# zafarrafii/REPET-Python

Measured on AMD Instinct MI355X. Metric: audio-seconds/sec (x real-time) for repet.sim, 44.1 kHz stereo, higher is better.
Workload: dtype f32 (similarity GEMM: f16x3 split of the fp32 unit rows, fp32 accumulate; median: exact selection on bit-sliced rank codes)

## Files before the change

### repet-python_amd/csrc/rank.hip

```cpp
#include "common.h"

namespace repet {

namespace {

__device__ __forceinline__ void cex(unsigned& a, unsigned& b) {
    const unsigned lo = a < b ? a : b, hi = a < b ? b : a;
    a = lo; b = hi;
}
__device__ __forceinline__ int phys(int i) { return i + ((i >> 5) << 2); }

template <int QHI, int QLO, int HB>
__device__ __forceinline__ void stages_high(unsigned (&r)[8][4]) {
#pragma unroll
    for (int q = QHI; q >= QLO; --q) {
        const int bit = 1 << (q - HB);
#pragma unroll
        for (int u = 0; u < 8; ++u)
            if (!(u & bit)) {
#pragma unroll
                for (int w = 0; w < 4; ++w) cex(r[u][w], r[u | bit][w]);
            }
    }
}
// ... 13 lines not shown
            const int src = (i0 ^ ((1 << (P - 1)) - 1)) & ~3;
            const uint4 v = *reinterpret_cast<const uint4*>(s + phys(src));
            r[u][0] = v.w; r[u][1] = v.z; r[u][2] = v.y; r[u][3] = v.x;
        } else {
            const uint4 v = *reinterpret_cast<const uint4*>(s + phys(i0));
            r[u][0] = v.x; r[u][1] = v.y; r[u][2] = v.z; r[u][3] = v.w;
        }
    }
    if (FLIP) __syncthreads();
    stages_high<QHI, QLO, HB>(r);
#pragma unroll
    for (int u = 0; u < 8; ++u)
        *reinterpret_cast<uint4*>(s + phys(base | (u << HB))) = make_uint4(r[u][0], r[u][1], r[u][2], r[u][3]);
}

template <int LOG2N, int P, int QHI>
struct HighTrips {
    static __device__ __forceinline__ void run(unsigned* s, int tid) {
        constexpr int QLO = QHI - 2 > 5 ? QHI - 2 : 5;
        trip_high<LOG2N, P, QHI, QLO, QHI == P - 1>(s, tid);
        if constexpr (QLO > 5) HighTrips<LOG2N, P, QLO - 1>::run(s, tid);
    }
};

__device__ __forceinline__ void stages_low(unsigned (&k)[32]) {
#pragma unroll
    for (int q = 4; q >= 0; --q) {
#pragma unroll
        for (int i = 0; i < 32; ++i)
            if (!(i & (1 << q))) cex(k[i], k[i | (1 << q)]);
    }
}

__device__ __forceinline__ void load_run(const unsigned* s, int tid, unsigned (&k)[32]) {
#pragma unroll
    for (int v = 0; v < 8; ++v) {
        const uint4 x = *reinterpret_cast<const uint4*>(s + phys(tid * 32 + v * 4));
        k[4 * v] = x.x; k[4 * v + 1] = x.y; k[4 * v + 2] = x.z; k[4 * v + 3] = x.w;
    }
}
__device__ __forceinline__ void store_run(unsigned* s, int tid, const unsigned (&k)[32]) {
#pragma unroll
    for (int v = 0; v < 8; ++v)
        *reinterpret_cast<uint4*>(s + phys(tid * 32 + v * 4)) = make_uint4(k[4 * v], k[4 * v + 1], k[4 * v + 2], k[4 * v + 3]);
}

template <int LOG2N, int P>
struct Phases {
    static __device__ __forceinline__ void run(unsigned* s, int tid, unsigned (&k)[32]) {
        HighTrips<LOG2N, P, P - 1>::run(s, tid);
        __syncthreads();
        load_run(s, tid, k);
        stages_low(k);
        store_run(s, tid, k);
        if constexpr (P < LOG2N) Phases<LOG2N, P + 1>::run(s, tid, k);
    }
};

}

constexpr int kColumnTileFrames = 32;
__global__ __launch_bounds__(256) void columns_from_rows_kernel(RankArgs a) {
    constexpr int TF = kColumnTileFrames;
    constexpr int kRounds = TF / 16;
    constexpr int kOutLanes = TF / 4;
    constexpr int kOutRounds = 64 * kOutLanes / 256;
    __shared__ float tile[TF][65];
    const int c = blockIdx.z, f0 = blockIdx.y * 64;
    const int64_t t0 = (int64_t)blockIdx.x * TF;
    const int tx = threadIdx.x & 15, ty = threadIdx.x >> 4;
    const float* in = a.V + c * a.chan_stride;
    float4 r[kRounds];
#pragma unroll
    for (int k = 0; k < kRounds; ++k) {
        const int64_t t = t0 + ty + 16 * k;
        r[k] = *reinterpret_cast<const float4*>(in + (t < a.T ? t : a.T - 1) * a.FS + f0 + 4 * tx);
    }
#pragma unroll
    for (int k = 0; k < kRounds; ++k) {
        const bool live = t0 + ty + 16 * k < a.T;
        float* row = tile[ty + 16 * k] + 4 * tx;
        row[0] = live ? r[k].x : 0.f; row[1] = live ? r[k].y : 0.f; row[2] = live ? r[k].z : 0.f; row[3] = live ? r[k].w : 0.f;
    }
    __syncthreads();
    float* out = a.Vs + ((int64_t)c * a.n_cols + f0) * a.vs_pitch;
    const int ox = threadIdx.x % kOutLanes, oy = threadIdx.x / kOutLanes;
    const int col0 = (oy & 3) + 32 * ((oy >> 2) & 1) + 4 * (threadIdx.x >> 6);
    if (t0 + 4 * ox < a.vs_pitch) {
#pragma unroll
        for (int k = 0; k < kOutRounds; ++k) {
            const int f = col0 + 16 * k;
            *reinterpret_cast<float4*>(out + (int64_t)f * a.vs_pitch + t0 + 4 * ox) =
                make_float4(tile[4 * ox][f], tile[4 * ox + 1][f], tile[4 * ox + 2][f], tile[4 * ox + 3][f]);
        }
    }
}

__global__ __launch_bounds__(256) void rows_from_code_columns_kernel(RankArgs a) {
    __shared__ unsigned tile[2][64][65];
    const int c = blockIdx.z, f0 = blockIdx.y * 128;
    const int64_t t0 = (int64_t)blockIdx.x * 128;
    const int tx = threadIdx.x & 63, ty = threadIdx.x >> 6;
    const unsigned* in = reinterpret_cast<const unsigned*>(a.codes + ((int64_t)c * a.n_cols + f0) * a.vs_pitch + t0);
    const bool in_range = t0 + 2 * tx < a.vs_pitch;
    unsigned r[32];
    const int txc = in_range ? tx : 0;
#pragma unroll
    for (int k = 0; k < 32; ++k) r[k] = in[(int64_t)(ty + 4 * k) * (a.vs_pitch / 2) + txc];
// ... 21 lines not shown
    for (int k = 0; k < 16; ++k)
        if (!(k & J)) {
            const unsigned t = ((x[k] >> J) ^ x[k + J]) & m;
            x[k + J] ^= t;
            x[k] ^= t << J;
        }
}
constexpr int kPlaneFrames = 32;
__global__ __launch_bounds__(1024) void code_planes_from_columns_kernel(RankArgs a) {
    constexpr int kPlaneColPitch = kPlaneFrames + 2, kPieces = kPlaneFrames / 8;
    extern __shared__ unsigned short plane_lds[];
    const int64_t t0 = (int64_t)blockIdx.x * kPlaneFrames;
    const int l0 = blockIdx.y * 32;
    const int bpc = a.n_cols >> 6, n_bits = a.n_channels * bpc;
    uint4 v[kPieces];
#pragma unroll
    for (int k = 0; k < kPieces; ++k) {
        const int i = threadIdx.x + 1024 * k, q = i / kPieces, piece = i % kPieces;
        const int b = q >> 5, l = l0 + (q & 31);
        const int64_t t = t0 + piece * 8;
        const bool in = b < n_bits && t < a.vs_pitch;
        const int c = in ? b / bpc : 0, f = in ? (b - c * bpc) * 64 + l : 0;
        v[k] = *reinterpret_cast<const uint4*>(a.codes + ((int64_t)c * a.n_cols + f) * a.vs_pitch + (in ? t : 0));
        if (!in) v[k] = make_uint4(0u, 0u, 0u, 0u);
    }
#pragma unroll
    for (int k = 0; k < kPieces; ++k) {
        const int i = threadIdx.x + 1024 * k, q = i / kPieces, piece = i % kPieces;
        unsigned* dst = reinterpret_cast<unsigned*>(plane_lds + q * kPlaneColPitch + piece * 8);
        dst[0] = v[k].x; dst[1] = v[k].y; dst[2] = v[k].z; dst[3] = v[k].w;
    }
    __syncthreads();
    const int l = threadIdx.x & 31;
#pragma unroll
    for (int k = 0; k < kPlaneFrames / 32; ++k) {
        const int tl = (threadIdx.x >> 5) + 32 * k;
        const int64_t t = t0 + tl;
        if (t >= a.T) continue;
        unsigned x[16];
#pragma unroll
        for (int b = 0; b < 16; ++b) {
            const unsigned lo = b < n_bits ? plane_lds[(b * 32 + l) * kPlaneColPitch + tl] - kRankCodeBase : 0u;
            const unsigned hi = b + 16 < n_bits ? plane_lds[((b + 16) * 32 + l) * kPlaneColPitch + tl] - kRankCodeBase : 0u;
            x[b] = (lo & 0xffffu) | (hi << 16);
        }
        plane_transpose_stage<8>(x); plane_transpose_stage<4>(x); plane_transpose_stage<2>(x); plane_transpose_stage<1>(x);
        unsigned* out = a.P + t * (int64_t)a.n_planes * 64 + l0 + l;
#pragma unroll
        for (int p = 0; p < 15; ++p)
            if (p < a.n_planes) out[p * 64] = x[p];
    }
}

#ifndef REPET_RANK_LEAF_BITS
#define REPET_RANK_LEAF_BITS 4
#endif
constexpr int rank_leaf_bits(int log2n) { return log2n >= 15 ? 5 : REPET_RANK_LEAF_BITS; }

template <int LOG2N>
__global__ __launch_bounds__((1 << LOG2N) / 32) void rank_columns_kernel(RankArgs a) {
    constexpr int N = 1 << LOG2N, THREADS = N / 32;
    extern __shared__ uint4 rank_lds[];
    unsigned* s = reinterpret_cast<unsigned*>(rank_lds);
    const int64_t col = blockIdx.x;
    const int tid = threadIdx.x;
    float* column = a.Vs + col * a.vs_pitch;
    const __amdgpu_buffer_rsrc_t v_rsrc = __builtin_amdgcn_make_buffer_rsrc(column, 0, (int)(a.T * 4), 0x00020000);
    unsigned k[32];
#pragma unroll
    for (int j = 0; j < 8; ++j) {
        const int t = 4 * tid + 4 * THREADS * j;
        const uint4 v = __builtin_bit_cast(uint4, __builtin_amdgcn_raw_buffer_load_b128(v_rsrc, t * 4, 0, 0));
        k[4 * j] = t < a.T ? v.x : 0x7f800000u;
        k[4 * j + 1] = t + 1 < a.T ? v.y : 0x7f800000u;
        k[4 * j + 2] = t + 2 < a.T ? v.z : 0x7f800000u;
        k[4 * j + 3] = t + 3 < a.T ? v.w : 0x7f800000u;
    }
#pragma unroll
    for (int p = 1; p <= 5; ++p) {
#pragma unroll
        for (int i2 = 0; i2 < 32; ++i2)
            if (!(i2 & (1 << (p - 1)))) cex(k[i2], k[i2 ^ ((1 << p) - 1)]);
#pragma unroll
        for (int q = p - 2; q >= 0; --q) {
#pragma unroll
            for (int i2 = 0; i2 < 32; ++i2)
                if (!(i2 & (1 << q))) cex(k[i2], k[i2 | (1 << q)]);
        }
    }
    store_run(s, tid, k);
    Phases<LOG2N, 6>::run(s, tid, k);
    unsigned orig[32], pos[32];
#pragma unroll
    for (int j = 0; j < 8; ++j) {
        const int t = 4 * tid + 4 * THREADS * j;
        const uint4 v = __builtin_bit_cast(uint4, __builtin_amdgcn_raw_buffer_load_b128(v_rsrc, t * 4, 0, 0));
        orig[4 * j] = v.x; orig[4 * j + 1] = v.y; orig[4 * j + 2] = v.z; orig[4 * j + 3] = v.w;
    }
    constexpr int R = rank_leaf_bits(LOG2N), kTreeLevels = LOG2N - R, kNodes = N >> R;
    unsigned* tree = s + (N + N / 8);
    __syncthreads();
#pragma unroll
    for (int n = tid; n < kNodes; n += THREADS)
        if (n > 0) {
            const int l = 31 - __clz(n), j = n - (1 << l);
            tree[n] = s[phys((((2 * j + 1) << (LOG2N - 1 - l))) - 1)];
        }
    __syncthreads();
    {
#pragma unroll
        for (int e = 0; e < 32; ++e) pos[e] = 1;
#pragma unroll 1
        for (int l = 0; l < kTreeLevels; ++l) {
#pragma unroll
            for (int e = 0; e < 32; ++e) {
                const unsigned probe = tree[pos[e]];
                pos[e] = 2 * pos[e] + (probe < orig[e] ? 1 : 0);
            }
        }
#pragma unroll
        for (int e = 0; e < 32; ++e) {
            const int g = pos[e] - kNodes;
            pos[e] = (g << R) + ((g >> (5 - R)) << 2) + (1 << (R - 1)) - 1;
        }
#pragma unroll
        for (int m = R - 1; m >= 0; --m) {
            const int step = 1 << m, d = m > 0 ? -((step >> 1) + 0) : 0;
#pragma unroll
            for (int e = 0; e < 32; ++e) {
                const unsigned probe = s[pos[e]];
                pos[e] += (probe < orig[e] ? step : 0) + d;
            }
        }
    }
#pragma unroll
    for (int e = 0; e < 32; ++e) pos[e] -= 4 * (pos[e] / 36);
    const __amdgpu_buffer_rsrc_t c_rsrc = __builtin_amdgcn_make_buffer_rsrc(a.codes + col * a.vs_pitch, 0, (int)(round_up(a.T, 4) * 2), 0x00020000);
#pragma unroll
    for (int j = 0; j < 8; ++j) {
        const int t = 4 * tid + 4 * THREADS * j;
        const unsigned lo = (kRankCodeBase + pos[4 * j]) | ((kRankCodeBase + pos[4 * j + 1]) << 16);
        const unsigned hi = (kRankCodeBase + pos[4 * j + 2]) | ((kRankCodeBase + pos[4 * j + 3]) << 16);
        __builtin_amdgcn_raw_buffer_store_b64(__builtin_bit_cast(__attribute__((__vector_size__(2 * sizeof(unsigned)))) unsigned, make_uint2(lo, hi)),
                                              c_rsrc, t * 2, 0, 0);
    }
    __syncthreads();
#pragma unroll
    for (int j = 0; j < 8; ++j) {
        const int t = 4 * tid + 4 * THREADS * j;
        if (t < a.vs_pitch) *reinterpret_cast<uint4*>(column + t) = *reinterpret_cast<const uint4*>(s + phys(t));
    }
}

__global__ void fill_rank_pad_rows_kernel(unsigned short* R, int64_t r_chan_stride, int64_t pad_row, int FS) {
    const int c = blockIdx.y;
    const int k = blockIdx.x * blockDim.x + threadIdx.x;
    if (k >= 2 * FS) return;
    R[c * r_chan_stride + pad_row * FS + k] = (k < FS) ? (unsigned short)0 : (unsigned short)0x7C00;
}

hipError_t launch_fill_rank_pad_rows(unsigned short* R, int64_t r_chan_stride, int32_t n_channels, int64_t pad_row,
                                     int32_t FS, hipStream_t s) {
    hipLaunchKernelGGL(fill_rank_pad_rows_kernel, dim3((unsigned)ceil_div(2 * FS, 256), (unsigned)n_channels), dim3(256), 0, s,
                       R, r_chan_stride, pad_row, FS);
    return hipGetLastError();
}

bool rank_columns_supported(int64_t T) { return T > kRankMinFrames && T <= kRankMaxFrames; }

template <int LOG2N>
static hipError_t launch_rank_n(const RankArgs& a, hipStream_t s, RankStepHook hook, void* user) {
    constexpr int N = 1 << LOG2N;
    constexpr int lds = (N + N / 8) * 4 + (N >> rank_leaf_bits(LOG2N)) * 4;
    hipError_t e = ensure_dynamic_lds(reinterpret_cast<const void*>(&rank_columns_kernel<LOG2N>), lds);
    if (e != hipSuccess) return e;
    const int64_t cols = (int64_t)a.n_channels * a.n_cols;
    hipLaunchKernelGGL(columns_from_rows_kernel, dim3((unsigned)ceil_div(a.vs_pitch, kColumnTileFrames), (unsigned)(a.n_cols / 64), (unsigned)a.n_channels),
                       dim3(256), 0, s, a);
    if (hook) hook(user, 0);
    hipLaunchKernelGGL(rank_columns_kernel<LOG2N>, dim3((unsigned)cols), dim3(N / 32), lds, s, a);
    if (hook) hook(user, 1);
    if (a.P) {
        constexpr int plane_lds_bytes = 1024 * (kPlaneFrames + 2) * 2;
        e = ensure_dynamic_lds(reinterpret_cast<const void*>(&code_planes_from_columns_kernel), plane_lds_bytes);
        if (e != hipSuccess) return e;
        hipLaunchKernelGGL(code_planes_from_columns_kernel, dim3((unsigned)ceil_div(a.T, kPlaneFrames), 2), dim3(1024), plane_lds_bytes, s, a);
        if (hook) hook(user, 2);
        return hipGetLastError();
    }
    hipLaunchKernelGGL(rows_from_code_columns_kernel, dim3((unsigned)ceil_div(a.vs_pitch, 128), (unsigned)(a.n_cols / 128), (unsigned)a.n_channels),
                       dim3(256), 0, s, a);
    if (hook) hook(user, 3);
    return hipGetLastError();
}

hipError_t launch_rank_columns(const RankArgs& a0, hipStream_t s, RankStepHook hook, void* user) {
    if (!rank_columns_supported(a0.T) || a0.n_cols <= 0 || (a0.n_cols & 127) || (a0.vs_pitch & 31) || (a0.FS & 1)) return hipErrorInvalidValue;
    if (a0.P && (a0.R || a0.n_planes != code_planes_for(a0.T) || a0.n_planes > 15 || a0.n_channels * (a0.n_cols >> 6) > 32)) return hipErrorInvalidValue;
    if (!a0.P && !a0.R) return hipErrorInvalidValue;
    RankArgs a = a0;
    if (a.T <= 2048) return launch_rank_n<11>(a, s, hook, user);
    if (a.T <= 4096) return launch_rank_n<12>(a, s, hook, user);
    if (a.T <= 8192) return launch_rank_n<13>(a, s, hook, user);
    if (a.T <= 16384) return launch_rank_n<14>(a, s, hook, user);
    return launch_rank_n<15>(a, s, hook, user);
}

}
```

### repet-python_amd/csrc/common.h

```cpp
#pragma once
#include <hip/hip_runtime.h>
#include <stdint.h>
#include "../../include/repet_hip.h"
#include <vector>

namespace repet {

constexpr int kWave = 64;
constexpr int kFreqAlign = 32;
constexpr int kTile = 128;
constexpr float kMaskEps = 2.220446049250313e-16f;

__host__ __device__ inline int64_t round_up(int64_t x, int64_t m) { return (x + m - 1) / m * m; }
__host__ __device__ inline int64_t ceil_div(int64_t x, int64_t m) { return (x + m - 1) / m; }

hipError_t ensure_dynamic_lds(const void* kernel, int bytes);


struct StftArgs {
    const float* audio; int64_t n_samples; int32_t n_channels;
    int64_t sample_offset;
    const float* window; const float2* twiddle;
    int32_t W, H; int64_t T; int32_t FS; int32_t centred;
    float2* X; float* V; int64_t chan_stride;
// ... 163 lines not shown
hipError_t launch_unit_rows_f64(const struct ExactSource& src, const PeakRefine* refine, hipStream_t s);
size_t local_maxima_scratch_bytes(int64_t n_rows, int32_t n_cols, int32_t d);

struct ExactSource {
    const float* hi; const float* lo; int64_t n_samples; int32_t n_channels; int64_t clip_stride;
    int64_t frame_sample0; int32_t W, H, F, FS;
    const double* window64; const double2* twiddle64;
    double* u64; int64_t u64_clip_stride; unsigned int* u64_gen; int64_t gen_clip_stride;
};
size_t local_maxima_exact_scratch_bytes(int32_t n_cols, int* grid_out = nullptr);
hipError_t launch_local_maxima_exact(const float* M, int64_t row0, int32_t n_cols, int64_t pitch, int32_t mode, float min_value,
                                     int32_t d, int32_t number, int32_t* idx, int32_t idx_pitch, int32_t* count, hipStream_t s,
                                     int64_t shift, const PeakRefine* refine, const PeakBatch* batch, const ExactSource& src,
                                     void* scratch);

__device__ __forceinline__ float soft_mask(float v, float model, int f, int cutoff) {
#ifdef REPET_IEEE_SQRT
    const float m = (fminf(v, model) + kMaskEps) / (v + kMaskEps);
#else
    const float q = fminf((model + kMaskEps) * __builtin_amdgcn_rcpf(v + kMaskEps), 1.0f);
    const float m = (model >= v) ? 1.0f : q;
#endif
    const float mm = (model != model) ? model : m;
    return (f >= 1 && f <= cutoff) ? 1.0f : mm;
}

struct MaskArgs {
    const float* V; int64_t chan_stride; int32_t n_channels; int64_t T; int32_t F, FS;
    float2* X; float* mask; int32_t cutoff;
    float* model; int64_t model_batch_stride, model_chan_stride;
    int64_t pad_row;
    int32_t n_batch; int64_t batch_stride;
    int64_t idx_batch_stride, cnt_batch_stride;
    int64_t frame0;
    int64_t frame_end;
    const unsigned short* R; int64_t r_chan_stride; const float* Vs; int64_t vs_pitch; int32_t n_rank_cols;
    const unsigned* P; int32_t n_planes;
    unsigned* median_codes;
    const int64_t* slot_start; int64_t slot_bias;
};
constexpr int kPadRows = 8;
constexpr int kMinIdxPitch = 128;
hipError_t launch_fill_pad_rows(float* V, int64_t chan_stride, int32_t n_channels, int64_t pad_row, int32_t FS,
                                hipStream_t s, float* Z = nullptr, int64_t z_stride = 0, int64_t z_count = 0, int32_t n_z = 0,
                                unsigned int* stats = nullptr, float* Z2 = nullptr);
hipError_t launch_mask_sim(const MaskArgs& m, const int32_t* idx, int32_t idx_pitch, const int32_t* count,
                           int64_t first_frame, int32_t max_count, hipStream_t s, int parts = 3, bool lookups_by_caller = false);
int median_network_instructions(int max_n, int* net_size);
int code_planes_for(int64_t T);
bool mask_sim_bits_supported(int64_t T, int32_t n_channels, int32_t n_cols, int32_t max_count);
int mask_sim_bits_instructions(int32_t max_count, int32_t n_planes);
hipError_t launch_mask_sim_bits(const MaskArgs& m, const int32_t* idx, int32_t idx_pitch, const int32_t* count, int32_t max_count,
                                unsigned n_launch, hipStream_t s);
hipError_t launch_mask_from_codes(const MaskArgs& m, const int32_t* count, hipStream_t s);
hipError_t launch_mask_adaptive(const MaskArgs& m, const int32_t* periods, int32_t order, hipStream_t s);
hipError_t launch_mask_period(const MaskArgs& m, const int32_t* period_dev, int32_t period_host,
                              int32_t min_period, hipStream_t s);

constexpr int kRankCodeBase = 0x0400;
constexpr int kRankMinFrames = 1024;
constexpr int kRankMaxFrames = 30720;
struct RankArgs {
    const float* V; int64_t chan_stride; int32_t n_channels; int64_t T; int32_t FS;
    int32_t n_cols;
    unsigned short* R; int64_t r_chan_stride;
    float* Vs; int64_t vs_pitch;
    unsigned short* codes;
    unsigned* P; int32_t n_planes;
};
bool rank_columns_supported(int64_t T);
std::vector<int> host_cpus_near_device(int dev);
typedef void (*RankStepHook)(void* user, int step);
hipError_t launch_rank_columns(const RankArgs& a, hipStream_t s, RankStepHook hook = nullptr, void* user = nullptr);
hipError_t launch_fill_rank_pad_rows(unsigned short* R, int64_t r_chan_stride, int32_t n_channels, int64_t pad_row,
                                     int32_t FS, hipStream_t s);

struct StagingRing {
    static constexpr int kSlots = 6;
    static constexpr size_t kSlotElems = (size_t)1 << 20;
    float* base = nullptr;
    float* base_lo = nullptr;
    float* lo_full = nullptr; size_t lo_full_elems = 0; hipEvent_t hi_done = nullptr, lo_done = nullptr; bool lo_in_flight = false;
    hipEvent_t event[kSlots] = {};
    bool busy[kSlots] = {};
    hipError_t ensure();
    hipError_t ensure_lo();
    hipError_t ensure_lo_full(size_t elems);
    void release();
    ~StagingRing();
};
hipError_t staged_upload(StagingRing& ring, const void* src, int dtype, float* dst, size_t count, hipStream_t s,
                         float* dst_lo = nullptr, bool* any_lo = nullptr, hipStream_t s_lo = nullptr, bool* not_finite = nullptr);
hipError_t staged_download(StagingRing& ring, const float* src, double* dst, size_t count, hipStream_t s);
hipError_t staged_upload_bytes(StagingRing& ring, const void* src, void* dst, size_t n_bytes, hipStream_t s);
const char* wav_parse(const void* file, int64_t n_bytes, ::repet_wav_info* info);
int wav_itemsize(const ::repet_wav_info& w);
hipError_t launch_decode_pcm(const void* raw, int format, int width, float* dst, int64_t n, hipStream_t s);
int64_t wav_float_header(unsigned char* out, int sampling_frequency, int n_channels, int64_t n_samples, int item_bytes);
void* host_alloc(size_t bytes);
void host_free(void* ptr);

hipError_t launch_convert_in(const void* src, int dtype, float* dst, int64_t count, hipStream_t s, float* dst_lo = nullptr);
hipError_t launch_convert_out(const float* src, double* dst, int64_t count, hipStream_t s);
hipError_t launch_foreground(const float* audio, const float* background, double* dst, int64_t count, hipStream_t s);
hipError_t launch_foreground_f32(const float* audio, const float* background, float* dst, int64_t count, hipStream_t s);
hipError_t launch_channel_mean(const float* audio, const float* background, int which, int n_channels, float* dst,
                               int64_t n_samples, hipStream_t s);
// ... 5 lines not shown
```

### repet-python_amd/csrc/engine_sim.hip

```cpp
#include "engine.h"

using namespace repet;
using namespace repet_eng;

namespace repet_eng {

float peak_refine_delta(int FS, bool f16_gram) {
    return (f16_gram ? 2.0f : 4.0f) * sqrtf((float)FS) * 5.9604645e-8f;
}

double peak_exact_delta2() {
    static const double v = [] { const char* off = getenv("REPET_PEAK_EXACT"); return (off && off[0] == '0') ? 0.0 : 2.5e-7; }();
    return v;
}

int ensure_stamps(repet_ctx* c, DevBuf& buf, size_t count) {
    if (buf.cap >= count * sizeof(unsigned int)) return REPET_OK;
    HIP_TRY(hipStreamSynchronize(c->stream));
    HIP_TRY(buf.ensure(count * sizeof(unsigned int)));
    HIP_TRY(hipMemsetAsync(buf.p, 0, buf.cap, c->stream));
    return REPET_OK;
}

int make_refine(repet_ctx* c, const float* unit_rows, int FS, double threshold, PeakRefine* rf, int64_t rows, int clips,
// ... 120 lines not shown
    const int64_t TS = round_up(T, 64);
    HIP_TRY(c->S.ensure((size_t)T * TS * sizeof(float)));
    const bool with_seg = local_maxima_segments_apply((int)T, p->sim_distance_frames, TS, 0, 1);
    const int seg_pitch = segment_pitch((int)TS);
    if (with_seg) HIP_TRY(c->seg.ensure((size_t)T * 3 * seg_pitch * sizeof(float)));
    float* seg = with_seg ? c->seg.as<float>() : nullptr;
    bool seg_written = false;
    RP_TRY(run_gram_full(c, c->Vn.as<float>(), T, g.FS, c->S.as<float>(), TS, true, split_in_stft(1), seg, seg_pitch, &seg_written));
    {
        const bool f16 = gram_f16_enabled();
        const int edge = (f16 && gram_big_enabled() && T >= 8 * gram_big_tile()) ? gram_big_tile() : kTile;
        const double n_tiles = 0.5 * (double)ceil_div(T, edge) * (double)(ceil_div(T, edge) + 1);
        mark(c, f16 ? "similarity_gemm_f16x3" : "similarity_gemm", 4.0 * g.F * T + 4.0 * T * T,
             (f16 ? 3.0 : 1.0) * 2.0 * g.FS * n_tiles * edge * edge);
    }
    if (seg && !seg_written) {
        HIP_TRY(launch_segment_maxima(c->S.as<float>(), T, (int)T, TS, seg, seg_pitch, c->stream));
        mark(c, "segment_maxima", 4.0 * T * T + 12.0 * T * seg_pitch, 0);
    }
    const int K = p->sim_number, KP = std::max(K, kMinIdxPitch);
    HIP_TRY(c->idx.ensure((size_t)T * KP * sizeof(int32_t)));
    HIP_TRY(c->cnt.ensure((size_t)T * sizeof(int32_t)));
    PeakRefine rf{};
    RP_TRY(make_refine(c, c->Vn.as<float>(), g.FS, p->sim_threshold, &rf, T, 1, (int)T, p->sim_distance_frames, T));
    {
        MaskArgs m = mask_args(c, g, p->cutoff_bins);
        static const bool overlap = [] { const char* e = getenv("REPET_RANK_OVERLAP"); return !(e && e[0] == '0'); }();
        const bool beside = use_rank && overlap;
        if (beside) {
            HIP_TRY(hipEventRecord(c->fork_event, c->stream));
            HIP_TRY(hipStreamWaitEvent(c->side_stream, c->fork_event, 0));
            RP_TRY(run_rank_columns(c, g, &m, c->side_stream, false, max_peaks));
            HIP_TRY(hipEventRecord(c->join_event, c->side_stream));
        }
        const size_t scratch = local_maxima_scratch_bytes(T, (int)T, p->sim_distance_frames);
        if (scratch > 0) HIP_TRY(c->peak_scratch.ensure(scratch));
        hipError_t e = launch_local_maxima(c->S.as<float>(), T, 0, (int)T, TS, 0, (float)p->sim_threshold,
                                           p->sim_distance_frames, K, c->idx.as<int32_t>(), KP, c->cnt.as<int32_t>(), c->stream, 0, &rf,
                                           nullptr, scratch > 0 ? c->peak_scratch.p : nullptr, nullptr, seg, seg_pitch);
        if (e == hipErrorInvalidValue) return fail(REPET_ERR_LIMIT, "sim: clip has too many frames for the peak-picking kernel's LDS row");
        HIP_TRY(e);
        if (use_rank && !beside) mark(c, "local_maxima_pass1", 12.0 * T * seg_pitch + 4.0 * K * T, 0);
        RP_TRY(run_exact_rows(c, tb, g, c->S.as<float>(), 0, (int)T, TS, 0, (float)p->sim_threshold, p->sim_distance_frames, K,
                              c->idx.as<int32_t>(), KP, c->cnt.as<int32_t>(), 0, rf, nullptr,
                              c->audio.as<float>() + c->clip_base * g.C, c->has_lo ? c->audio_lo.as<float>() + c->clip_base * g.C : nullptr,
                              N, 0, -(int64_t)(g.W / 2), T, 1));
        if (beside) {
            HIP_TRY(hipStreamWaitEvent(c->stream, c->join_event, 0));
            mark(c, "peaks+rank_columns", 4.0 * T * T + 4.0 * K * T + (4.0 + 4.0 + 8.0 + 4.0 + 2.0 + 2.0 + 2.0) * (g.F - 1) * (double)g.T * g.C, 0);
        } else {
            mark(c, use_rank ? "local_maxima_level2" : "local_maxima", use_rank ? 0.0 : 4.0 * T * T + 4.0 * K * T, 0);
            if (use_rank) RP_TRY(run_rank_columns(c, g, &m, c->stream, true, max_peaks));
        }
        HIP_TRY(launch_mask_sim(m, c->idx.as<int32_t>(), KP, c->cnt.as<int32_t>(), 0, max_peaks, c->stream, 3, m.P != nullptr));
        c->last_median_path = m.P ? 2 : m.R ? 1 : 0;
        c->last_FS = g.FS; c->last_chan_stride = g.chan_stride;
        if (m.P) {
            mark(c, "mask_sim_select", 256.0 * m.n_planes * (K + 1.0) * T + 4.0 * (g.F - 1) * T * g.C, 0);
            HIP_TRY(launch_mask_from_codes(m, c->cnt.as<int32_t>(), c->stream));
            mark(c, "mask_sim", (4.0 + 4.0 + 8.0 + (c->mask_plane ? 4.0 : 16.0)) * (g.F - 1) * T * g.C, 0);
        } else
            mark(c, "mask_sim", (4.0 + 4.0 * K + (c->mask_plane ? 4.0 : 16.0)) * g.F * T * g.C, 0);
    }
    RP_TRY(run_istft(c, g, tb, g.W - g.H, N, 0, false, 0, 0));
    c->last_T = T; c->last_idx_rows = T; c->last_idx_pitch = KP; c->last_idx_number = K;
    return REPET_OK;
}

int exec_simonline(repet_ctx* c, const repet_params* p) {
    MaskPlaneScope plane(c, mask_plane_wanted(MaskKind::sim_float));
    Tables* tb = nullptr;
    RP_TRY(get_tables(c, p->window_length, &tb));
    const int64_t N = c->n_samples;
    const int W = p->window_length, H = p->step_length, B = p->buffer_frames;
    if (B < 1) return fail(REPET_ERR_BAD_ARG, "buffer length must be >= 1 frame");
    if (N < (int64_t)(B - 2) * H + W)
        return fail(REPET_ERR_TOO_SHORT, "operands could not be broadcast together (signal shorter than the buffer)");
    const int64_t T = repet_frame_count(N, W, H, 0);
    const Geo g = make_geo(W, H, T, c->n_channels);
    if (p->sim_number < 1) return fail(REPET_ERR_BAD_ARG, "similarity_number must be >= 1");
    const int nb = c->clip_loop ? 1 : c->n_clips;
    RP_TRY(ensure_spectra(c, g, true, false, nb));
    RP_TRY(run_stft(c, g, tb, 0, N, 0, true, false, nb, N));
    const int LP = (int)round_up(B, 64);
    const int64_t mean_stride = g.Tpad * g.FS, band_stride = g.Tpad * LP, spec_stride = (int64_t)g.C * g.chan_stride;
    HIP_TRY(c->band.ensure((size_t)nb * band_stride * sizeof(float)));
    RP_TRY(run_gram_band(c, c->Vn.as<float>(), T, g.FS, c->band.as<float>(), B, LP, true, nb, mean_stride, band_stride, split_in_stft(nb), true));
    const int peak_mode = c->band_lookback ? 2 : 1;
    mark(c, c->band_on_f16 ? "similarity_band_f16x3" : "similarity_band", nb * (4.0 * g.F * T + 4.0 * T * B), nb * 2.0 * g.F * (double)T * B);
    const int K = p->sim_number, KP = std::max(K, kMinIdxPitch);
    const int64_t rows = T >= B ? T - B + 1 : 0;
    const int64_t rows_alloc = std::max<int64_t>(rows, 1);
    HIP_TRY(c->idx.ensure((size_t)nb * rows_alloc * KP * sizeof(int32_t)));
    HIP_TRY(c->cnt.ensure((size_t)nb * rows_alloc * sizeof(int32_t)));
    PeakRefine rf{};
    RP_TRY(make_refine(c, c->Vn.as<float>(), g.FS, p->sim_threshold, &rf, rows, nb, B, p->sim_distance_frames, T));
    const PeakBatch pb{nb, band_stride, rows_alloc * KP, rows_alloc, mean_stride};
    hipError_t e = launch_local_maxima(c->band.as<float>(), rows, B - 1, B, LP, peak_mode, (float)p->sim_threshold,
                                       p->sim_distance_frames, K, c->idx.as<int32_t>(), KP, c->cnt.as<int32_t>(), c->stream, 0, &rf,
                                       nb > 1 ? &pb : nullptr);
    if (e == hipErrorInvalidValue) return fail(REPET_ERR_LIMIT, "simonline: buffer too long for the peak-picking kernel");
    HIP_TRY(e);
    if (rows > 0)
        RP_TRY(run_exact_rows(c, tb, g, c->band.as<float>(), B - 1, B, LP, peak_mode, (float)p->sim_threshold, p->sim_distance_frames, K,
                              c->idx.as<int32_t>(), KP, c->cnt.as<int32_t>(), 0, rf, nb > 1 ? &pb : nullptr,
                              c->audio.as<float>() + c->clip_base * g.C, c->has_lo ? c->audio_lo.as<float>() + c->clip_base * g.C : nullptr,
                              N, N * g.C, 0, T, nb));
    mark(c, "local_maxima", nb * (4.0 * rows * B + 4.0 * K * rows), 0);
    const int max_peaks = (int)std::min<int64_t>(K, ceil_div(B, p->sim_distance_frames + 1));
    if (c->nonfinite_passes() && B > 1) {
        for (int b = 0; b < nb; ++b)
            for (int ch = 0; ch < g.C; ++ch)
// ... 28 lines not shown
```

### repet-python_amd/csrc/mask_bits.hip

```cpp
#include "common.h"

namespace repet {

namespace {

template <int IMM>
__device__ __forceinline__ unsigned bitop3(unsigned a, unsigned b, unsigned c) { return __builtin_amdgcn_bitop3_b32(a, b, c, IMM); }
__device__ __forceinline__ unsigned bs_xor3(unsigned a, unsigned b, unsigned c) { return bitop3<0x96>(a, b, c); }
__device__ __forceinline__ unsigned bs_maj(unsigned a, unsigned b, unsigned c) { return bitop3<0xE8>(a, b, c); }
__device__ __forceinline__ unsigned bs_or3(unsigned a, unsigned b, unsigned c) { return bitop3<0xFE>(a, b, c); }
__device__ __forceinline__ unsigned bs_and3(unsigned a, unsigned b, unsigned c) { return bitop3<0x80>(a, b, c); }
__device__ __forceinline__ unsigned bs_andn(unsigned a, unsigned b) { return bitop3<0x30>(a, b, b); }
__device__ __forceinline__ unsigned bs_keep(unsigned a, unsigned b, unsigned s) { return bitop3<0x60>(a, b, s); }
__device__ __forceinline__ unsigned bs_borrow(unsigned r, unsigned c, unsigned bw) { return bitop3<0x8E>(r, c, bw); }
__device__ __forceinline__ unsigned bs_sel(unsigned s, unsigned x, unsigned y) { return bitop3<0xCA>(s, x, y); }
__device__ __forceinline__ unsigned bs_or_andn(unsigned d, unsigned a, unsigned b) { return bitop3<0xF4>(d, a, b); }
#include "bitslice_count.inc"

constexpr int bit_length(int v) { return v <= 0 ? 0 : 1 + bit_length(v >> 1); }

template <int J>
__device__ __forceinline__ void transpose16_stage(unsigned (&x)[16]) {
    constexpr unsigned m = J == 8 ? 0x00FF00FFu : J == 4 ? 0x0F0F0F0Fu : J == 2 ? 0x33333333u : 0x55555555u;
#pragma unroll
// ... 97 lines not shown
                prev = c3;
            }
            const unsigned bw = diff[kR];
            unsigned all = diff[0];
#pragma unroll
            for (int d = 1; d <= kR; ++d) all &= diff[d];
            const unsigned part = all & bw & even;
            const unsigned s1 = bw, s2 = bs_sel(D, any2, bw & ~part);
            D = bs_or_andn(D, s1, s2);
#pragma unroll
            for (int d = 0; d < kR; ++d) r1[d] = bs_sel(bw, r1[d], diff[d]);
            dec[0][lane] = s1; dec[1][lane] = s2;
            lu[0][p][lane] = ~s1; lu[1][p][lane] = ~s2;
            __builtin_amdgcn_s_setprio(0);
        }
        __syncthreads();
        const unsigned s1 = dec[0][lane], s2 = dec[1][lane];
        const int next = lane * 4 + (p > 0 ? p - 1 : 0) * (kRowWords * 4);
#pragma unroll
        for (int k = 0; k < H; ++k) {
            A1[k] = bs_keep(A1[k], B[k], s1);
            A2[k] = bs_keep(A2[k], B[k], s2);
            B[k] = (unsigned)__builtin_amdgcn_raw_buffer_load_b32(rsrc, next + off[k], 0, 0);
        }
    }
    const int n_bits = a.n_channels << bpc_shift;
    unsigned own[NP];
#pragma unroll
    for (int p = 0; p < NP; ++p) own[p] = (unsigned)__builtin_amdgcn_raw_buffer_load_b32(rsrc, (unsigned)(t * kRowBytes) + lane * 4, p * (kRowWords * 4), 0);
    unsigned need = 0u, x[16];
    const unsigned pick = 0x0C040C00u + 0x00010001u * w;
#pragma unroll
    for (int p = 0; p < 16; ++p) {
        if (p < NP) {
            const unsigned lo = lu[0][p][lane], hi = lu[1][p][lane];
            need = bs_borrow(lo, own[p], need);
            x[p] = __builtin_amdgcn_perm(hi, lo, pick);
        } else x[p] = 0u;
    }
    transpose16_halves(x);
    const __amdgpu_buffer_rsrc_t c_rsrc = __builtin_amdgcn_make_buffer_rsrc(a.median_codes, 0, (int)(a.n_channels * a.chan_stride * 4), 0x00020000);
#pragma unroll
    for (int j = 0; j < 8; ++j) {
        const int b = 8 * w + j;
        if (b < n_bits) {
            const int c = b >> bpc_shift, fb = b - (c << bpc_shift);
            const int row = (int)(c * a.chan_stride + t * a.FS) + fb * 64;
            const unsigned flag = ((need >> b) & 1u) << 15;
            __builtin_amdgcn_raw_buffer_store_b32(x[j] | flag, c_rsrc, lane * 4, row * 4, 2);
        }
    }
}

__global__ __launch_bounds__(256) void mask_from_codes_kernel(MaskArgs a, const int* __restrict__ count, int n_quads) {
    const int lane = threadIdx.x & 63, wave = __builtin_amdgcn_readfirstlane(threadIdx.x >> 6);
    const int nfb = a.n_rank_cols >> 7;
    const int b = blockIdx.x, xcd = b & 7, i = b >> 3;
    const int combo = (i / n_quads) * 8 + xcd;
    if (combo >= a.n_channels * nfb) return;
    const int c = combo / nfb, fb = combo % nfb;
    const int64_t t_end = a.frame_end > 0 ? a.frame_end : a.T;
    const int64_t t = a.frame0 + 4 * (int64_t)(i % n_quads) + wave;
    if (t >= t_end) return;
    const int f0 = fb * 128 + 2 * lane;
    const float* vs = a.Vs + ((int64_t)c * a.n_rank_cols + f0) * a.vs_pitch;
    const int64_t o = c * a.chan_stride + t * a.FS + f0;
    const int n = count[t];
    typedef float f2 __attribute__((ext_vector_type(2)));
    typedef float f4 __attribute__((ext_vector_type(4)));
    typedef unsigned u2 __attribute__((ext_vector_type(2)));
    const f2 v_nt = __builtin_nontemporal_load(reinterpret_cast<const f2*>(a.V + o));
    const u2 c_nt = __builtin_nontemporal_load(reinterpret_cast<const u2*>(a.median_codes + o));
    const float2 v_own = make_float2(v_nt.x, v_nt.y);
    const uint2 cw = make_uint2(c_nt.x, c_nt.y);
    float4 x_own = make_float4(0.f, 0.f, 0.f, 0.f);
    if (a.X) { const f4 x_nt = __builtin_nontemporal_load(reinterpret_cast<const f4*>(a.X + o)); x_own = make_float4(x_nt.x, x_nt.y, x_nt.z, x_nt.w); }
    float a0 = v_own.x, b0 = v_own.x, a1 = v_own.y, b1 = v_own.y;
    const bool need0 = cw.x & 0x8000u, need1 = cw.y & 0x8000u;
    if (need0) { a0 = vs[cw.x & 0x7fffu]; b0 = vs[cw.x >> 16]; }
    if (need1) { a1 = vs[a.vs_pitch + (cw.y & 0x7fffu)]; b1 = vs[a.vs_pitch + (cw.y >> 16)]; }
    float med0 = need0 ? ((n & 1) ? a0 : 0.5f * (a0 + b0)) : v_own.x;
    float med1 = need1 ? ((n & 1) ? a1 : 0.5f * (a1 + b1)) : v_own.y;
    if (n <= 0) med0 = med1 = __uint_as_float(0x7fc00000u);
    const float m0 = soft_mask(v_own.x, med0, f0, a.cutoff), m1 = soft_mask(v_own.y, med1, f0 + 1, a.cutoff);
    if (a.mask) *reinterpret_cast<float2*>(a.mask + o) = make_float2(m0, m1);
    if (a.X) *reinterpret_cast<float4*>(a.X + o) = make_float4(x_own.x * m0, x_own.y * m0, x_own.z * m1, x_own.w * m1);
}

template <int H>
hipError_t launch_bits_h(const MaskArgs& m, const int32_t* idx, int32_t idx_pitch, const int32_t* count, unsigned n_launch, int bpc_shift,
                         hipStream_t s) {
#define REPET_BITS_CASE(NP) case NP: hipLaunchKernelGGL((mask_sim_bits_kernel<H, NP>), dim3(8 * ((n_launch + 7) / 8)), dim3(256), 0, s, m, idx, idx_pitch, count, bpc_shift); break;
    switch (m.n_planes) {
        REPET_BITS_CASE(11) REPET_BITS_CASE(12) REPET_BITS_CASE(13) REPET_BITS_CASE(14) REPET_BITS_CASE(15)
        default: return hipErrorInvalidValue;
    }
#undef REPET_BITS_CASE
    return hipGetLastError();
}

}

int code_planes_for(int64_t T) { int np = 11; while (((int64_t)1 << np) < T) ++np; return np; }

bool mask_sim_bits_supported(int64_t T, int32_t n_channels, int32_t n_cols, int32_t max_count) {
    const int bpc = n_cols >> 6;
    return rank_columns_supported(T) && n_cols > 0 && (n_cols & 127) == 0 && (bpc & (bpc - 1)) == 0 && n_channels * bpc <= 32 &&
           max_count <= 128 && code_planes_for(T) <= 15;
}

int mask_sim_bits_instructions(int32_t max_count, int32_t n_planes) {
    const int h = max_count <= 100 ? 25 : 32;
    const int count = h == 25 ? BitsliceCount<25>::kInstructions : BitsliceCount<32>::kInstructions;
    const int kr = bit_length(4 * h);
    const int per_wave = 2 * h + count + h / 2 + 2 * h, leader = 3 * 2 * kr + 4 * kr + 6;
    return (4 * per_wave + leader) * n_planes;
}

hipError_t launch_mask_sim_bits(const MaskArgs& m, const int32_t* idx, int32_t idx_pitch, const int32_t* count, int32_t max_count,
                                unsigned n_launch, hipStream_t s) {
    if (!m.P || !mask_sim_bits_supported(m.T, m.n_channels, m.n_rank_cols, max_count) || m.n_planes != code_planes_for(m.T) ||
        idx_pitch < 128 || !m.median_codes || (int64_t)m.n_channels * m.chan_stride * 4 >= ((int64_t)1 << 31))
        return hipErrorInvalidValue;
    int bpc_shift = 0;
    while ((64 << bpc_shift) < m.n_rank_cols) ++bpc_shift;
    return max_count <= 100 ? launch_bits_h<25>(m, idx, idx_pitch, count, n_launch, bpc_shift, s)
                            : launch_bits_h<32>(m, idx, idx_pitch, count, n_launch, bpc_shift, s);
}

hipError_t launch_mask_from_codes(const MaskArgs& m, const int32_t* count, hipStream_t s) {
    const int64_t t_end = m.frame_end > 0 ? m.frame_end : m.T;
    if (!m.median_codes || !m.Vs || t_end <= m.frame0 || (m.n_rank_cols & 127)) return hipErrorInvalidValue;
    const int n_quads = (int)ceil_div(t_end - m.frame0, 4);
    const int combos = m.n_channels * (m.n_rank_cols >> 7);
    hipLaunchKernelGGL(mask_from_codes_kernel, dim3((unsigned)(8 * ceil_div(combos, 8) * n_quads)), dim3(256), 0, s, m, count, n_quads);
    return hipGetLastError();
}

}
```

Measured before the change: 217,300.

## Store sorted column in Eytzinger layout from registers for branchless rank search

```diff
diff --git a/repet-python_amd/csrc/rank.hip b/repet-python_amd/csrc/rank.hip
--- a/repet-python_amd/csrc/rank.hip
+++ b/repet-python_amd/csrc/rank.hip
@@ -89,8 +89,10 @@
         __syncthreads();
         load_run(s, tid, k);
         stages_low(k);
-        store_run(s, tid, k);
-        if constexpr (P < LOG2N) Phases<LOG2N, P + 1>::run(s, tid, k);
+        if constexpr (P < LOG2N) {
+            store_run(s, tid, k);
+            Phases<LOG2N, P + 1>::run(s, tid, k);
+        }
     }
 };
 
@@ -218,11 +220,6 @@
     }
 }
 
-#ifndef REPET_RANK_LEAF_BITS
-#define REPET_RANK_LEAF_BITS 4
-#endif
-constexpr int rank_leaf_bits(int log2n) { return log2n >= 15 ? 5 : REPET_RANK_LEAF_BITS; }
-
 template <int LOG2N>
 __global__ __launch_bounds__((1 << LOG2N) / 32) void rank_columns_kernel(RankArgs a) {
     constexpr int N = 1 << LOG2N, THREADS = N / 32;
@@ -256,6 +253,20 @@
     }
     store_run(s, tid, k);
     Phases<LOG2N, 6>::run(s, tid, k);
+    __syncthreads();
+    {
+        unsigned* lv = s + N / 2 + 16 * tid;
+#pragma unroll
+        for (int v = 0; v < 4; ++v) *reinterpret_cast<uint4*>(lv + 4 * v) = make_uint4(k[8 * v], k[8 * v + 2], k[8 * v + 4], k[8 * v + 6]);
+        lv = s + N / 4 + 8 * tid;
+        *reinterpret_cast<uint4*>(lv) = make_uint4(k[1], k[5], k[9], k[13]);
+        *reinterpret_cast<uint4*>(lv + 4) = make_uint4(k[17], k[21], k[25], k[29]);
+        *reinterpret_cast<uint4*>(s + N / 8 + 4 * tid) = make_uint4(k[3], k[11], k[19], k[27]);
+        *reinterpret_cast<uint2*>(s + N / 16 + 2 * tid) = make_uint2(k[7], k[23]);
+        s[N / 32 + tid] = k[15];
+        const int m = tid + 1;
+        s[m == THREADS ? 0 : (THREADS + m) >> (__ffs(m))] = k[31];
+    }
     unsigned orig[32], pos[32];
 #pragma unroll
     for (int j = 0; j < 8; ++j) {
@@ -263,50 +274,24 @@
         const uint4 v = __builtin_bit_cast(uint4, __builtin_amdgcn_raw_buffer_load_b128(v_rsrc, t * 4, 0, 0));
         orig[4 * j] = v.x; orig[4 * j + 1] = v.y; orig[4 * j + 2] = v.z; orig[4 * j + 3] = v.w;
     }
-    constexpr int R = rank_leaf_bits(LOG2N), kTreeLevels = LOG2N - R, kNodes = N >> R;
-    unsigned* tree = s + (N + N / 8);
-    __syncthreads();
-#pragma unroll
-    for (int n = tid; n < kNodes; n += THREADS)
-        if (n > 0) {
-            const int l = 31 - __clz(n), j = n - (1 << l);
-            tree[n] = s[phys((((2 * j + 1) << (LOG2N - 1 - l))) - 1)];
-        }
-    __syncthreads();
-    {
-#pragma unroll
-        for (int e = 0; e < 32; ++e) pos[e] = 1;
+    __syncthreads();
+#pragma unroll
+    for (int e = 0; e < 32; ++e) pos[e] = 1;
 #pragma unroll 1
-        for (int l = 0; l < kTreeLevels; ++l) {
-#pragma unroll
-            for (int e = 0; e < 32; ++e) {
-                const unsigned probe = tree[pos[e]];
-                pos[e] = 2 * pos[e] + (probe < orig[e] ? 1 : 0);
-            }
-        }
+    for (int l = 0; l < LOG2N; ++l) {
 #pragma unroll
         for (int e = 0; e < 32; ++e) {
-            const int g = pos[e] - kNodes;
-            pos[e] = (g << R) + ((g >> (5 - R)) << 2) + (1 << (R - 1)) - 1;
-        }
-#pragma unroll
-        for (int m = R - 1; m >= 0; --m) {
-            const int step = 1 << m, d = m > 0 ? -((step >> 1) + 0) : 0;
-#pragma unroll
-            for (int e = 0; e < 32; ++e) {
-                const unsigned probe = s[pos[e]];
-                pos[e] += (probe < orig[e] ? step : 0) + d;
-            }
-        }
-    }
-#pragma unroll
-    for (int e = 0; e < 32; ++e) pos[e] -= 4 * (pos[e] / 36);
+            const unsigned probe = s[pos[e]];
+            asm("v_cmp_lt_u32 vcc, %1, %2\n\tv_addc_co_u32 %0, vcc, %0, %0, vcc" : "+v"(pos[e]) : "v"(probe), "v"(orig[e]) : "vcc");
+        }
+    }
     const __amdgpu_buffer_rsrc_t c_rsrc = __builtin_amdgcn_make_buffer_rsrc(a.codes + col * a.vs_pitch, 0, (int)(round_up(a.T, 4) * 2), 0x00020000);
 #pragma unroll
     for (int j = 0; j < 8; ++j) {
         const int t = 4 * tid + 4 * THREADS * j;
-        const unsigned lo = (kRankCodeBase + pos[4 * j]) | ((kRankCodeBase + pos[4 * j + 1]) << 16);
-        const unsigned hi = (kRankCodeBase + pos[4 * j + 2]) | ((kRankCodeBase + pos[4 * j + 3]) << 16);
+        constexpr unsigned kBias = kRankCodeBase - N;
+        const unsigned lo = (kBias + pos[4 * j]) | ((kBias + pos[4 * j + 1]) << 16);
+        const unsigned hi = (kBias + pos[4 * j + 2]) | ((kBias + pos[4 * j + 3]) << 16);
         __builtin_amdgcn_raw_buffer_store_b64(__builtin_bit_cast(__attribute__((__vector_size__(2 * sizeof(unsigned)))) unsigned, make_uint2(lo, hi)),
                                               c_rsrc, t * 2, 0, 0);
     }
@@ -314,7 +299,11 @@
 #pragma unroll
     for (int j = 0; j < 8; ++j) {
         const int t = 4 * tid + 4 * THREADS * j;
-        if (t < a.vs_pitch) *reinterpret_cast<uint4*>(column + t) = *reinterpret_cast<const uint4*>(s + phys(t));
+        const uint2 odd = *reinterpret_cast<const uint2*>(s + N / 2 + t / 2);
+        const unsigned r2 = s[N / 4 + t / 4];
+        const int m = t / 4 + 1;
+        const unsigned r4 = s[m == N / 4 ? 0 : (N / 4 + m) >> (__ffs(m))];
+        if (t < a.vs_pitch) *reinterpret_cast<uint4*>(column + t) = make_uint4(odd.x, r2, odd.y, r4);
     }
 }
 
@@ -337,7 +326,7 @@
 template <int LOG2N>
 static hipError_t launch_rank_n(const RankArgs& a, hipStream_t s, RankStepHook hook, void* user) {
     constexpr int N = 1 << LOG2N;
-    constexpr int lds = (N + N / 8) * 4 + (N >> rank_leaf_bits(LOG2N)) * 4;
+    constexpr int lds = (N + N / 8) * 4;
     hipError_t e = ensure_dynamic_lds(reinterpret_cast<const void*>(&rank_columns_kernel<LOG2N>), lds);
     if (e != hipSuccess) return e;
     const int64_t cols = (int64_t)a.n_channels * a.n_cols;
```

Result: faster. 220,300 (median of 6 runs) (+1.4%).

## Fold the leftover frequency bin's median into the mask-from-codes kernel

Applied to the files above, without the earlier changes.

```diff
diff --git a/repet-python_amd/csrc/common.h b/repet-python_amd/csrc/common.h
--- a/repet-python_amd/csrc/common.h
+++ b/repet-python_amd/csrc/common.h
@@ -239,7 +239,8 @@
 int mask_sim_bits_instructions(int32_t max_count, int32_t n_planes);
 hipError_t launch_mask_sim_bits(const MaskArgs& m, const int32_t* idx, int32_t idx_pitch, const int32_t* count, int32_t max_count,
                                 unsigned n_launch, hipStream_t s);
-hipError_t launch_mask_from_codes(const MaskArgs& m, const int32_t* count, hipStream_t s);
+hipError_t launch_mask_from_codes(const MaskArgs& m, const int32_t* count, hipStream_t s, const int32_t* idx = nullptr,
+                                  int32_t idx_pitch = 0);
 hipError_t launch_mask_adaptive(const MaskArgs& m, const int32_t* periods, int32_t order, hipStream_t s);
 hipError_t launch_mask_period(const MaskArgs& m, const int32_t* period_dev, int32_t period_host,
                               int32_t min_period, hipStream_t s);
diff --git a/repet-python_amd/csrc/engine_sim.hip b/repet-python_amd/csrc/engine_sim.hip
--- a/repet-python_amd/csrc/engine_sim.hip
+++ b/repet-python_amd/csrc/engine_sim.hip
@@ -196,12 +196,14 @@
             mark(c, use_rank ? "local_maxima_level2" : "local_maxima", use_rank ? 0.0 : 4.0 * T * T + 4.0 * K * T, 0);
             if (use_rank) RP_TRY(run_rank_columns(c, g, &m, c->stream, true, max_peaks));
         }
-        HIP_TRY(launch_mask_sim(m, c->idx.as<int32_t>(), KP, c->cnt.as<int32_t>(), 0, max_peaks, c->stream, 3, m.P != nullptr));
+        const bool lone_in_lookups = m.P != nullptr && m.frame0 == 0 && m.frame_end <= 0;
+        HIP_TRY(launch_mask_sim(m, c->idx.as<int32_t>(), KP, c->cnt.as<int32_t>(), 0, max_peaks, c->stream, lone_in_lookups ? 1 : 3,
+                                m.P != nullptr));
         c->last_median_path = m.P ? 2 : m.R ? 1 : 0;
         c->last_FS = g.FS; c->last_chan_stride = g.chan_stride;
         if (m.P) {
             mark(c, "mask_sim_select", 256.0 * m.n_planes * (K + 1.0) * T + 4.0 * (g.F - 1) * T * g.C, 0);
-            HIP_TRY(launch_mask_from_codes(m, c->cnt.as<int32_t>(), c->stream));
+            HIP_TRY(launch_mask_from_codes(m, c->cnt.as<int32_t>(), c->stream, lone_in_lookups ? c->idx.as<int32_t>() : nullptr, KP));
             mark(c, "mask_sim", (4.0 + 4.0 + 8.0 + (c->mask_plane ? 4.0 : 16.0)) * (g.F - 1) * T * g.C, 0);
         } else
             mark(c, "mask_sim", (4.0 + 4.0 * K + (c->mask_plane ? 4.0 : 16.0)) * g.F * T * g.C, 0);
diff --git a/repet-python_amd/csrc/mask_bits.hip b/repet-python_amd/csrc/mask_bits.hip
--- a/repet-python_amd/csrc/mask_bits.hip
+++ b/repet-python_amd/csrc/mask_bits.hip
@@ -173,10 +173,65 @@
     }
 }
 
-__global__ __launch_bounds__(256) void mask_from_codes_kernel(MaskArgs a, const int* __restrict__ count, int n_quads) {
+__device__ __forceinline__ void lone_bin_of_frame(const MaskArgs& a, const int* __restrict__ idx, int idx_pitch,
+                                                  const int* __restrict__ count, int64_t t, int ch0, int lane) {
+    const int f = a.F - 1;
+    const int n = __builtin_amdgcn_readfirstlane(count[t]);
+    const int* list = idx + t * (int64_t)idx_pitch;
+    const bool has0 = lane < n, has1 = lane + 64 < n;
+    const int e0 = has0 ? list[lane] : 0, e1 = has1 ? list[lane + 64] : 0;
+    const int n_ch = ch0 + 1 < a.n_channels ? 2 : 1;
+    unsigned u0[2], u1[2];
+    float v_own[2];
+    float2 x_own[2];
+#pragma unroll
+    for (int q = 0; q < 2; ++q) {
+        const int ch = q < n_ch ? ch0 + q : ch0;
+        const float* Vc = a.V + ch * a.chan_stride;
+        u0[q] = has0 ? __float_as_uint(Vc[(int64_t)e0 * a.FS + f]) ^ 0x80000000u : ~0u;
+        u1[q] = has1 ? __float_as_uint(Vc[(int64_t)e1 * a.FS + f]) ^ 0x80000000u : ~0u;
+        v_own[q] = Vc[t * a.FS + f];
+        x_own[q] = make_float2(0.f, 0.f);
+        if (a.X && lane == 0) x_own[q] = a.X[ch * a.chan_stride + t * a.FS + f];
+    }
+#pragma unroll
+    for (int q = 0; q < 2; ++q) {
+        if (q >= n_ch) break;
+        auto value_of_rank = [&](int r) -> float {
+            unsigned P = 0u;
+#pragma unroll
+            for (int b = 31; b >= 0; --b) {
+                const unsigned T = P | (1u << b);
+                const int below = __popcll(__ballot(u0[q] < T)) + __popcll(__ballot(u1[q] < T));
+                P = below <= r ? T : P;
+            }
+            return __uint_as_float(P ^ 0x80000000u);
+        };
+        float med = __uint_as_float(0x7fc00000u);
+        if (n > 0) {
+            const float lo = value_of_rank((n - 1) >> 1);
+            med = (n & 1) ? lo : 0.5f * (lo + value_of_rank(n >> 1));
+        }
+        if (lane == 0) {
+            const int64_t o = (ch0 + q) * a.chan_stride + t * a.FS + f;
+            const float m = soft_mask(v_own[q], med, f, a.cutoff);
+            if (a.mask) a.mask[o] = m;
+            if (a.X) a.X[o] = make_float2(mul_rounded(x_own[q].x, m), mul_rounded(x_own[q].y, m));
+        }
+    }
+}
+
+__global__ __launch_bounds__(256) void mask_from_codes_kernel(MaskArgs a, const int* __restrict__ count, int n_quads,
+                                                              const int* __restrict__ idx, int idx_pitch, int n_lone) {
     const int lane = threadIdx.x & 63, wave = __builtin_amdgcn_readfirstlane(threadIdx.x >> 6);
+    if ((int)blockIdx.x < n_lone) {
+        const int64_t t = a.frame0 + 4 * (int64_t)(blockIdx.x % n_quads) + wave;
+        const int ch0 = 2 * (int)(blockIdx.x / n_quads);
+        if (t < (a.frame_end > 0 ? a.frame_end : a.T) && ch0 < a.n_channels) lone_bin_of_frame(a, idx, idx_pitch, count, t, ch0, lane);
+        return;
+    }
     const int nfb = a.n_rank_cols >> 7;
-    const int b = blockIdx.x, xcd = b & 7, i = b >> 3;
+    const int b = blockIdx.x - n_lone, xcd = b & 7, i = b >> 3;
     const int combo = (i / n_quads) * 8 + xcd;
     if (combo >= a.n_channels * nfb) return;
     const int c = combo / nfb, fb = combo % nfb;
@@ -249,12 +304,15 @@
                             : launch_bits_h<32>(m, idx, idx_pitch, count, n_launch, bpc_shift, s);
 }
 
-hipError_t launch_mask_from_codes(const MaskArgs& m, const int32_t* count, hipStream_t s) {
+hipError_t launch_mask_from_codes(const MaskArgs& m, const int32_t* count, hipStream_t s, const int32_t* idx, int32_t idx_pitch) {
     const int64_t t_end = m.frame_end > 0 ? m.frame_end : m.T;
     if (!m.median_codes || !m.Vs || t_end <= m.frame0 || (m.n_rank_cols & 127)) return hipErrorInvalidValue;
+    if (idx && (idx_pitch < 128 || m.F != m.n_rank_cols + 1)) return hipErrorInvalidValue;
     const int n_quads = (int)ceil_div(t_end - m.frame0, 4);
     const int combos = m.n_channels * (m.n_rank_cols >> 7);
-    hipLaunchKernelGGL(mask_from_codes_kernel, dim3((unsigned)(8 * ceil_div(combos, 8) * n_quads)), dim3(256), 0, s, m, count, n_quads);
+    const int n_lone = idx ? (int)(8 * ceil_div((int64_t)ceil_div(m.n_channels, 2) * n_quads, 8)) : 0;
+    hipLaunchKernelGGL(mask_from_codes_kernel, dim3((unsigned)(n_lone + 8 * ceil_div(combos, 8) * n_quads)), dim3(256), 0, s, m, count, n_quads,
+                       idx, idx_pitch, n_lone);
     return hipGetLastError();
 }
 
```

Measured after the change: 211,700 before, 210,800 after. Within noise of the previous version (-0.4%).
